# olegroshka/vae-channel-dynamics

Hardware: AMD Instinct MI355X
Metric: images/sec SDXL-VAE train step @256x256 (tracking on) (higher is better)
Workload: dtype f32

## Files before the change

vae-channel-dynamics_amd/csrc/conv3_upwino.hip:

```cpp
#include "wino_common.h"
#include <type_traits>
#include <algorithm>

#ifndef VAE_UPW_PRIO
#define VAE_UPW_PRIO 1
#endif

namespace {

constexpr int UTH = 4, UTW = 8;
constexpr int UTL = UTH * UTW;
static_assert(UTL == wino::TILES, "spill_acc");
constexpr int UBK = 8;
constexpr int NPOS = 9;
constexpr int UNT = 512;
constexpr int UNB = 2;
constexpr int USV = NPOS * UTL * UBK;
constexpr int UHF = (UTH + 2) * (UTW + 2);
constexpr int UHD = (2 * UTH + 2) * (2 * UTW + 2);
constexpr int USH = UHD * UBK;
constexpr int UMLD = 33;
constexpr int USM = NPOS * UTL * UMLD;
constexpr int UP_LDS = (USM > 2 * USV + 2 * USH ? USM : 2 * USV + 2 * USH) * 4;

__global__ __launch_bounds__(256) void upwino_weights_kernel(const float* __restrict__ W, int N, int K, int dgrad, int64_t sn, int64_t sk, int64_t st,
                                                             float* __restrict__ U) {
  const int64_t i = (int64_t)blockIdx.x * 256 + threadIdx.x;
  if (i >= (int64_t)N * K) return;
  const int k = (int)(i % K), n = (int)(i / K);
  float g[3][3];
  wino::u_gather(W, n, k, dgrad, sn, sk, st, g);
  float t[3][3];
#pragma unroll
  for (int b = 0; b < 3; ++b) {
    t[0][b] = g[0][b];
    t[1][b] = (g[0][b] + g[2][b]) + g[1][b];
    t[2][b] = g[2][b];
  }
  float* o = wino::u_out<NPOS>(U, N, n, k);
#pragma unroll
  for (int a = 0; a < 3; ++a) {
    wino::u_at(o, N, a * 3 + 0) = t[a][0];
    wino::u_at(o, N, a * 3 + 1) = (t[a][0] + t[a][2]) + t[a][1];
    wino::u_at(o, N, a * 3 + 2) = t[a][2];
  }
}

template <bool DG>
__global__ __launch_bounds__(UNT, 4) void conv3_upwino_kernel(vae_igemm_args p, const float* __restrict__ U, int tiles_x, int tiles_y, int xcd_sp) {
  constexpr int WBN = 32 * UNB;
  constexpr int HW_ = DG ? 2 * UTW + 2 : UTW + 2;
  constexpr int HP = DG ? UHD : UHF;
  __shared__ __attribute__((aligned(16))) float wsm[UP_LDS / 4];
  float* const sV = wsm;
  float* const sH = wsm + 2 * USV;

  const int tid = threadIdx.x, lane = tid & 63, wave = tid >> 6;
  const int xw0 = (blockIdx.x & 1) * 2;
  const bool extra = wave == xw0 || wave == xw0 + 1;
  const int xnb = wave - xw0;
  const int lr = lane & 31, lh = lane >> 5;
  const vae_conv_geom g = p.g;
  const int tilesN = (p.N + WBN - 1) / WBN;
  const wino::TileId wg = wino::tile_of_workgroup(blockIdx.x, tilesN, tiles_x, tiles_y, xcd_sp);
  const int b = wg.b;
  const int y0 = wg.ty * UTH, x0 = wg.tx * UTW, n0 = wg.tn * WBN;
  const int nsteps = p.K / UBK;

  const bool hrole = tid < 2 * HP;
  const int hp = tid >> 1, hq = tid & 1;
  const int hy = (DG ? 2 * y0 : y0) - 1 + hp / HW_, hx = (DG ? 2 * x0 : x0) - 1 + hp % HW_;
  const bool hin = hrole && ((unsigned)hy < (unsigned)g.Hs) && ((unsigned)hx < (unsigned)g.Ws);
  const auto rsA = VAE_BUF_RSRC(p.A + (int64_t)b * g.Hs * g.Ws * g.Cs, (size_t)g.Hs * g.Ws * g.Cs * 4u);
  const unsigned hbase = hin ? (unsigned)(((hy * g.Ws + hx) * g.Cs + hq * 4) * 4) : BUF_OOB;
  f32x4 rh = {0.f, 0.f, 0.f, 0.f};
  auto load_halo_into = [&](int step, f32x4& h) {
    const bool ok = hin && step < nsteps;
    h = VAE_BUF_LOAD4(rsA, ok ? hbase + (unsigned)(step * UBK * 4) : BUF_OOB);
  };
  auto store_halo_from = [&](float* dst, const f32x4& h) {
    if (hrole) *reinterpret_cast<f32x4*>(&dst[hp * UBK + hq * 4]) = h;
  };

  const bool vrole = tid < 256;
  const int vt = (tid >> 3) & 31, vc = tid & 7;
  const int vorg = DG ? ((2 * (vt >> 3)) * HW_ + 2 * (vt & 7)) * UBK + vc : ((vt >> 3) * HW_ + (vt & 7)) * UBK + vc;
  auto write_v = [&](const float* sHc, float* dst) {
    if (!vrole) return;
    float r[3][DG ? 4 : 3];
    if (!DG) {
      float d[3][3];
#pragma unroll
      for (int i = 0; i < 3; ++i)
#pragma unroll
        for (int j = 0; j < 3; ++j) d[i][j] = sHc[vorg + (i * HW_ + j) * UBK];
#pragma unroll
      for (int j = 0; j < 3; ++j) {
        r[0][j] = d[0][j] - d[1][j];
        r[1][j] = d[1][j];
        r[2][j] = d[1][j] - d[2][j];
      }
#pragma unroll
      for (int a = 0; a < 3; ++a) {
        dst[((a * 3 + 0) * UTL + vt) * UBK + vc] = r[a][0] - r[a][1];
        dst[((a * 3 + 1) * UTL + vt) * UBK + vc] = r[a][1];
        dst[((a * 3 + 2) * UTL + vt) * UBK + vc] = r[a][1] - r[a][2];
      }
    } else {
      float d[4][4];
#pragma unroll
      for (int i = 0; i < 4; ++i)
#pragma unroll
        for (int j = 0; j < 4; ++j) d[i][j] = sHc[vorg + (i * HW_ + j) * UBK];
#pragma unroll
      for (int j = 0; j < 4; ++j) {
        r[0][j] = d[0][j] - d[2][j];
        r[1][j] = d[1][j] + d[2][j];
        r[2][j] = d[1][j] - d[3][j];
      }
#pragma unroll
      for (int a = 0; a < 3; ++a) {
        dst[((a * 3 + 0) * UTL + vt) * UBK + vc] = r[a][0] - r[a][2];
        dst[((a * 3 + 1) * UTL + vt) * UBK + vc] = r[a][1] + r[a][2];
        dst[((a * 3 + 2) * UTL + vt) * UBK + vc] = r[a][1] - r[a][3];
      }
    }
  };

  const auto rsU = VAE_BUF_RSRC(U, wino::u_bytes(nsteps, NPOS, p.N));
  unsigned bvo[UNB];
#pragma unroll
  for (int q = 0; q < UNB; ++q) bvo[q] = (n0 + q * 32 + lr < p.N) ? wino::u_frag(n0 + q * 32 + lr, lh) : BUF_OOB;
  const unsigned bpos = wino::u_pos_bytes(p.N);
  const unsigned bvx = extra ? bvo[xnb & 1] : BUF_OOB;
  f32x4 bq[UNB + 1];
  auto load_b1 = [&](int step, int i) {
    const int st = min(step, nsteps - 1);
    const unsigned so = __builtin_amdgcn_readfirstlane((unsigned)(st * NPOS + (i < UNB ? wave : 8)) * bpos);
    bq[i] = __builtin_bit_cast(f32x4, __builtin_amdgcn_raw_buffer_load_b128(rsU, i < UNB ? bvo[i < UNB ? i : 0] : bvx, so, 0));
  };

  f32x16 acc[UNB], accx;
#pragma unroll
  for (int nb = 0; nb < UNB; ++nb)
#pragma unroll
    for (int e = 0; e < 16; ++e) acc[nb][e] = 0.f;
#pragma unroll
  for (int e = 0; e < 16; ++e) accx[e] = 0.f;

#pragma unroll
  for (int i = 0; i <= UNB; ++i) load_b1(0, i);
  {
    f32x4 h0, h1;
    load_halo_into(0, h0);
    load_halo_into(1, h1);
    load_halo_into(2, rh);
    store_halo_from(sH, h0);
    store_halo_from(sH + USH, h1);
  }
  __syncthreads();
  write_v(sH, sV);
  __syncthreads();
  auto multiply = [&](const float* cV, int s) {
    const f32x4 a4 = *reinterpret_cast<const f32x4*>(&cV[(wave * UTL + lr) * UBK + 4 * lh]);
    f32x4 ax = a4;
    if (extra) ax = *reinterpret_cast<const f32x4*>(&cV[(8 * UTL + lr) * UBK + 4 * lh]);
#pragma unroll
    for (int nb = 0; nb < UNB; ++nb) {
#pragma unroll
      for (int e = 0; e < 4; ++e) acc[nb] = __builtin_amdgcn_mfma_f32_32x32x2f32(a4[e], bq[nb][e], acc[nb], 0, 0, 0);
      __builtin_amdgcn_sched_barrier(0);
      load_b1(s + 1, nb);
      __builtin_amdgcn_sched_barrier(0);
    }
    if (extra) {
#pragma unroll
      for (int e = 0; e < 4; ++e) accx = __builtin_amdgcn_mfma_f32_32x32x2f32(ax[e], bq[UNB][e], accx, 0, 0, 0);
    }
    __builtin_amdgcn_sched_barrier(0);
    load_b1(s + 1, UNB);
    __builtin_amdgcn_sched_barrier(0);
  };
  auto stage_next = [&](int s, int par) {
    if (s + 1 < nsteps) write_v(sH + (par ^ 1) * USH, sV + (par ^ 1) * USV);
    store_halo_from(sH + par * USH, rh);
    load_halo_into(s + 3, rh);
  };
  auto step = [&](int s, int par, auto first_c) {
    const float* cV = sV + par * USV;
    if (decltype(first_c)::value) {
      stage_next(s, par);
      __builtin_amdgcn_sched_barrier(0);
      multiply(cV, s);
    } else {
      multiply(cV, s);
      __builtin_amdgcn_sched_barrier(0);
      stage_next(s, par);
    }
    __syncthreads();
  };
  auto run = [&](auto first_c) {
    int s = 0;
    for (; s + 1 < nsteps; s += 2) {
      step(s, 0, first_c);
      step(s + 1, 1, first_c);
    }
    if (s < nsteps) step(s, 0, first_c);
  };
#if VAE_UPW_PRIO
  if (DG && __builtin_amdgcn_readfirstlane(tid) >= 256) __builtin_amdgcn_s_setprio(1);
#endif
  if (wave < 4) run(std::true_type{});
  else run(std::false_type{});
#if VAE_UPW_PRIO
  if (DG) __builtin_amdgcn_s_setprio(0);
#endif

  float* const sM = wsm;
  const size_t obytes = (size_t)g.Ho * g.Wo * p.ldc * 4u;
  const auto rsC = VAE_BUF_RSRC(p.C + (int64_t)b * g.Ho * g.Wo * p.ldc, obytes);
#pragma unroll
  for (int nb = 0; nb < UNB; ++nb) {
    if (nb > 0) __syncthreads();
    wino::spill_acc(sM, wave, UMLD, acc[nb], lr, lh);
    if (wave == xw0 + nb) wino::spill_acc(sM, 8, UMLD, accx, lr, lh);
    __syncthreads();
    {
#pragma unroll
      for (int rnd = 0; rnd < 2; ++rnd) {
        const int co = tid & 31, tile = (tid >> 5) + 16 * rnd;
        const int col = n0 + nb * 32 + co;
        float m[9];
#pragma unroll
        for (int pos = 0; pos < 9; ++pos) m[pos] = sM[(pos * UTL + tile) * UMLD + co];
        const int oy = y0 + (tile >> 3), ox = x0 + (tile & 7);
        if (!DG) {
          const float bv = (p.bias && col < p.N) ? p.bias[col] : 0.f;
          float h[2][3];
#pragma unroll
          for (int j = 0; j < 3; ++j) {
            h[0][j] = m[0 * 3 + j] + m[1 * 3 + j];
            h[1][j] = m[1 * 3 + j] - m[2 * 3 + j];
          }
#pragma unroll
          for (int a = 0; a < 2; ++a) {
            const float yv[2] = {h[a][0] + h[a][1], h[a][1] - h[a][2]};
#pragma unroll
            for (int bb = 0; bb < 2; ++bb) {
              const int py = 2 * oy + a, px = 2 * ox + bb;
              const unsigned off = (col < p.N && py < g.Ho && px < g.Wo) ? (unsigned)(((py * g.Wo + px) * p.ldc + col) * 4) : BUF_OOB;
              __builtin_amdgcn_raw_buffer_store_b32(__builtin_bit_cast(unsigned, yv[bb] + bv), rsC, off, 0, 0);
            }
          }
        } else {
          const float h0 = (m[0] + m[3]) - m[6], h1 = (m[1] + m[4]) - m[7], h2 = (m[2] + m[5]) - m[8];
          const float v = (h0 + h1) - h2;
          const unsigned off = (col < p.N && oy < g.Ho && ox < g.Wo) ? (unsigned)(((oy * g.Wo + ox) * p.ldc + col) * 4) : BUF_OOB;
          __builtin_amdgcn_raw_buffer_store_b32(__builtin_bit_cast(unsigned, v), rsC, off, 0, 0);
        }
      }
    }
  }
}

}

bool conv3_upwino_eligible(const vae_igemm_args& a) {
  const vae_conv_geom& g = a.g;
  if (!wino::conv_eligible_common(a, NPOS) || a.xf != VAE_XF_NONE) return false;
  if (a.track != nullptr || a.res != nullptr || a.gstat != nullptr || a.a_bf16 || a.res_bf16) return false;
  int Hl, Wl;
  if (g.mode == VAE_MODE_UP2X) {
    if (g.Ho != 2 * g.Hs || g.Wo != 2 * g.Ws || a.sk != 1) return false;
    Hl = g.Hs; Wl = g.Ws;
  } else if (g.mode == VAE_MODE_UP2X_DGRAD) {
    if (g.Hs != 2 * g.Ho || g.Ws != 2 * g.Wo || a.sn != 1 || a.bias != nullptr) return false;
    Hl = g.Ho; Wl = g.Wo;
  } else {
    return false;
  }
  if (Hl % UTH != 0 || Wl % UTW != 0 || a.K % UBK != 0 || a.K < 64 || a.K > 1024 || a.N < 32 || a.N % 4 != 0 || g.Cs < a.K) return false;
  return true;
}

int launch_upwino_weights(const vae_igemm_args& a, float* U, hipStream_t st) {
  return wino::launch_weights(upwino_weights_kernel, a, a.g.mode == VAE_MODE_UP2X_DGRAD, U, st);
}

int launch_conv3_upwino(const vae_igemm_args& a, const float* U, hipStream_t st) {
  const vae_conv_geom& g = a.g;
  const bool dg = g.mode == VAE_MODE_UP2X_DGRAD;
  const int Hl = dg ? g.Ho : g.Hs, Wl = dg ? g.Wo : g.Ws;
  const int tx = Wl / UTW, ty = Hl / UTH;
  const int tilesN = (a.N + 32 * UNB - 1) / (32 * UNB);
  const int64_t nt = (int64_t)tilesN * tx * ty * g.B;
  if (nt > 0x7fffffffLL) return VAE_EINVAL;
  constexpr size_t xcd_u = (size_t)4 << 20;
  const int xcd_sp = wino::xcd_spatial(tilesN, wino::u_bytes(a.K / UBK, NPOS, a.N), xcd_u, (int64_t)tx * ty * g.B);
  if (dg) hipLaunchKernelGGL((conv3_upwino_kernel<true>), dim3((unsigned)nt), dim3(UNT), 0, st, a, U, tx, ty, xcd_sp);
  else hipLaunchKernelGGL((conv3_upwino_kernel<false>), dim3((unsigned)nt), dim3(UNT), 0, st, a, U, tx, ty, xcd_sp);
  return 0;
}
```

vae-channel-dynamics_amd/csrc/skinny.hip:

```cpp
#include "bf16_frag.h"
#include <algorithm>

namespace {

constexpr int TP = 128;
constexpr int NT = 256;
constexpr int TAPS_MAX = 9;

__device__ __forceinline__ void stage_small(const vae_conv_geom& g, const float* __restrict__ S, int Cs_small, int K, int m0,
                                            int mrows, f32x4* __restrict__ sI) {
  const int hw = g.Ho * g.Wo;
  const size_t sbytes = (size_t)g.B * g.Hs * g.Ws * Cs_small * 4u;
  const auto rsS = VAE_BUF_RSRC(S, sbytes < BUF_MAX ? sbytes : BUF_MAX);
  for (int e = threadIdx.x; e < TP * g.taps; e += NT) {
    const int row = e / g.taps, tap = e - row * g.taps;
    const int m = m0 + row;
    const int b = m / hw, rem = m - b * hw;
    const int y = rem / g.Wo, x = rem - y * g.Wo;
    const int kh = (g.taps == 9) ? tap / 3 : 0, kw = (g.taps == 9) ? tap - kh * 3 : 0;
    int sy = 0, sx = 0;
    const bool ok = (m < mrows) && src_pixel(g, y, x, kh, kw, sy, sx);
    const unsigned base = ok ? (unsigned)(((b * g.Hs + sy) * g.Ws + sx) * Cs_small) * 4u : BUF_OOB;
    f32x4 v = {0.f, 0.f, 0.f, 0.f};
#pragma unroll
    for (int s = 0; s < 4; ++s)
      if (s < K) v[s] = __builtin_bit_cast(float, __builtin_amdgcn_raw_buffer_load_b32(rsS, ok ? base + 4u * s : BUF_OOB, 0, 0));
    sI[e] = v;
  }
}

__global__ __launch_bounds__(NT) void conv_smallk_kernel(vae_igemm_args p) {
  __shared__ f32x4 sI[TP * TAPS_MAX];
  const vae_conv_geom g = p.g;
  const int tid = threadIdx.x, lane = tid & 127, half = tid >> 7;
  const int m0 = blockIdx.x * TP;
  const int n = blockIdx.y * 128 + lane;
  const bool nok = n < p.N;
  stage_small(g, p.A, g.Cs, p.K, m0, p.M, sI);

  float w[TAPS_MAX][4];
#pragma unroll
  for (int t = 0; t < TAPS_MAX; ++t)
#pragma unroll
    for (int s = 0; s < 4; ++s)
      w[t][s] = (nok && t < g.taps && s < p.K) ? p.W[(int64_t)n * p.sn + (int64_t)t * p.st + (int64_t)s * p.sk] : 0.f;
  const float bv = (p.bias && nok) ? p.bias[n] : 0.f;
  const bool cbf = p.out_bf16 != 0;
  const size_t obytes = (size_t)p.M * p.ldc * (cbf ? 2u : 4u);
  const auto rsC = VAE_BUF_RSRC(p.C, obytes);
  __syncthreads();

  float tsum = 0.f;
#pragma unroll 4
  for (int i = 0; i < TP / 2; ++i) {
    const int row = half + 2 * i;
    float acc = bv;
#pragma unroll
    for (int t = 0; t < TAPS_MAX; ++t) {
      if (t < g.taps) {
        const f32x4 v = sI[row * g.taps + t];
#pragma unroll
        for (int s = 0; s < 4; ++s) acc += v[s] * w[t][s];
      }
    }
    const int m = m0 + row;
    const bool ok = nok && m < p.M;
    buf_store1_elem(rsC, cbf, ok ? m * p.ldc + n : -1, acc);
    const float stored = cbf ? (float)(__bf16)acc : acc;
    tsum += ok ? fabsf(stored) : 0.f;
  }
  if (p.track) {
    __syncthreads();
    float* red = reinterpret_cast<float*>(sI);
    red[tid] = tsum;
    __syncthreads();
    if (half == 0 && nok) p.track[(int64_t)blockIdx.x * p.N + n] = red[lane] + red[128 + lane];
  }
}

template <bool SMALL_X, int XF>
__global__ __launch_bounds__(NT) void wgrad_smallk_kernel(vae_wgrad_args p, vae_conv_geom gs, int ntiles) {
  __shared__ f32x4 sI[TP * TAPS_MAX + 32];
  const int tid = threadIdx.x, lane = tid & 127, half = tid >> 7;
  const int split = blockIdx.x;
  const int ch = blockIdx.y * 128 + lane;
  const int wide = SMALL_X ? p.M : p.N, narrow = SMALL_X ? p.N : p.M;
  const bool chok = ch < wide;
  const float* __restrict__ V = SMALL_X ? p.dY : p.X;
  const float* __restrict__ S = SMALL_X ? p.X : p.dY;
  const int ldv = SMALL_X ? p.ldy : p.g.Cs, lds_ = SMALL_X ? p.g.Cs : p.ldy;
  const int npixv = gs.B * gs.Ho * gs.Wo;
  const int hwv = gs.Ho * gs.Wo;
  const bool vbf = (SMALL_X ? p.y_bf16 : p.x_bf16) != 0;
  const size_t vbytes = (size_t)npixv * ldv * (vbf ? 2u : 4u);
  const auto rsV = VAE_BUF_RSRC(V, vbytes < BUF_MAX ? vbytes : BUF_MAX);

  float acc[TAPS_MAX][4];
#pragma unroll
  for (int t = 0; t < TAPS_MAX; ++t)
#pragma unroll
    for (int s = 0; s < 4; ++s) acc[t][s] = 0.f;
  float vsum = 0.f;
  f32x4 ssum = {0.f, 0.f, 0.f, 0.f};
  int xb = -1;
  float xsc = 1.f, xsh = 0.f;

  const int per = (ntiles + p.nsplit - 1) / p.nsplit;
  const int tbeg = split * per, tend = min(ntiles, tbeg + per);
  for (int tile = tbeg; tile < tend; ++tile) {
    const int m0 = tile * TP;
    __syncthreads();
    stage_small(gs, S, lds_, narrow, m0, npixv, sI);
    __syncthreads();
#pragma unroll 4
    for (int i = 0; i < TP / 2; ++i) {
      const int row = half + 2 * i;
      const int m = m0 + row;
      const bool ok = chok && m < npixv;
      float v = buf_load1_elem(rsV, vbf, ok ? m * ldv + ch : -1);
      if (XF != VAE_XF_NONE) {
        const int b = min(m, npixv - 1) / hwv;
        if (b != xb) {
          xb = b;
          xsc = chok ? p.scale[(int64_t)b * p.g.Cs + ch] : 0.f;
          xsh = chok ? p.shift[(int64_t)b * p.g.Cs + ch] : 0.f;
        }
        float u = v * xsc + xsh;
        if (XF == VAE_XF_AFFINE_SILU) u = silu_f(u);
        v = ok ? u : 0.f;
      }
      if (SMALL_X) vsum += v;
#pragma unroll
      for (int t = 0; t < TAPS_MAX; ++t) {
        if (t < gs.taps) {
          const f32x4 sv = sI[row * gs.taps + t];
#pragma unroll
          for (int s = 0; s < 4; ++s) acc[t][s] += v * sv[s];
          if (!SMALL_X && t == gs.taps / 2) ssum += sv;
        }
      }
    }
  }

  __syncthreads();
  float* red = reinterpret_cast<float*>(sI);
  if (half == 1) {
#pragma unroll
    for (int t = 0; t < TAPS_MAX; ++t)
#pragma unroll
      for (int s = 0; s < 4; ++s) red[lane * 36 + t * 4 + s] = acc[t][s];
    if (SMALL_X) red[128 * 36 + lane] = vsum;
    else if (lane == 0) {
#pragma unroll
      for (int s = 0; s < 4; ++s) red[128 * 36 + s] = ssum[s];
    }
  }
  __syncthreads();
  if (half == 0) {
    const int64_t ld = (int64_t)gs.taps * p.N;
    float* __restrict__ O = (p.nsplit == 1 ? p.out : p.partial + (int64_t)split * p.M * ld);
    if (chok) {
#pragma unroll
      for (int t = 0; t < TAPS_MAX; ++t)
#pragma unroll
        for (int s = 0; s < 4; ++s)
          if (t < gs.taps && s < narrow) {
            const float r = acc[t][s] + red[lane * 36 + t * 4 + s];
            if (SMALL_X) O[(int64_t)ch * ld + (int64_t)t * p.N + s] = p.alpha * r;
            else O[(int64_t)s * ld + (int64_t)t * p.N + ch] = p.alpha * r;
          }
    }
    if (p.bias_partial) {
      if (SMALL_X) {
        if (chok) p.bias_partial[(int64_t)split * p.M + ch] = vsum + red[128 * 36 + lane];
      } else if (blockIdx.y == 0 && lane < p.M) {
        p.bias_partial[(int64_t)split * p.M + lane] = ssum[lane] + red[128 * 36 + lane];
      }
    }
  }
}

}

bool conv_smallk_eligible(const vae_igemm_args& a) {
  const vae_conv_geom& g = a.g;
  return a.K <= 4 && a.batch == 1 && a.xf == VAE_XF_NONE && a.res == nullptr && a.alpha == 1.0f && g.taps <= TAPS_MAX &&
         g.mode != VAE_MODE_DGRAD_S2 && (size_t)a.M * a.ldc * 4u < BUF_MAX && (size_t)g.B * g.Hs * g.Ws * g.Cs * 4u < BUF_MAX;
}
int launch_conv_smallk(const vae_igemm_args& a, hipStream_t st) {
  dim3 grid((unsigned)((a.M + TP - 1) / TP), (unsigned)((a.N + 127) / 128));
  hipLaunchKernelGGL(conv_smallk_kernel, grid, dim3(NT), 0, st, a);
  return 0;
}

int wgrad_smallk_kind(const vae_wgrad_args& a) {
  const vae_conv_geom& g = a.g;
  if (a.batch != 1 || g.taps > TAPS_MAX) return 0;
  if ((size_t)a.npix * a.ldy * 4u >= BUF_MAX || (size_t)g.B * g.Hs * g.Ws * g.Cs * 4u >= BUF_MAX) return 0;
  if (a.N <= 4 && a.xf == VAE_XF_NONE && (g.mode == VAE_MODE_FWD || g.mode == VAE_MODE_UP2X)) return 1;
  if (a.M <= 4 && g.mode == VAE_MODE_FWD && g.stride == 1 && g.Ho == g.Hs && g.Wo == g.Ws &&
      ((g.taps == 9 && g.pad_t == 1 && g.pad_l == 1) || (g.taps == 1 && g.pad_t == 0 && g.pad_l == 0)))
    return 2;
  return 0;
}
int wgrad_smallk_tiles(const vae_wgrad_args& a) { return (int)(((int64_t)a.g.B * a.g.Ho * a.g.Wo + TP - 1) / TP); }
static vae_conv_geom wgrad_smallk_geom(const vae_wgrad_args& a, int kind) {
  vae_conv_geom gs = a.g;
  if (kind == 2) {
    gs.mode = VAE_MODE_DGRAD;
    gs.Cs = a.ldy;
  }
  return gs;
}
int launch_wgrad_thin_bf16(const vae_wgrad_args& a, int kind, const vae_conv_geom& gs, int ntiles, hipStream_t st);
int launch_wgrad_thin(const vae_wgrad_args& a, hipStream_t st) {
  const int kind = wgrad_smallk_kind(a);
  return launch_wgrad_thin_bf16(a, kind, wgrad_smallk_geom(a, kind), wgrad_smallk_tiles(a), st);
}

int launch_wgrad_smallk(const vae_wgrad_args& a, hipStream_t st) {
  const int kind = wgrad_smallk_kind(a);
  const int ntiles = wgrad_smallk_tiles(a);
  const vae_conv_geom gs = wgrad_smallk_geom(a, kind);
  const int wide = kind == 1 ? a.M : a.N;
  dim3 grid((unsigned)a.nsplit, (unsigned)((wide + 127) / 128));
#define WSK(SX, XFV) hipLaunchKernelGGL((wgrad_smallk_kernel<SX, XFV>), grid, dim3(NT), 0, st, a, gs, ntiles)
  if (kind == 1) WSK(true, VAE_XF_NONE);
  else if (a.xf == VAE_XF_NONE) WSK(false, VAE_XF_NONE);
  else if (a.xf == VAE_XF_AFFINE) WSK(false, VAE_XF_AFFINE);
  else WSK(false, VAE_XF_AFFINE_SILU);
#undef WSK
  return 0;
}

namespace {

constexpr int NTH = 4, NTW = 32, NHW = NTW + 2, NHP = (NTH + 2) * NHW;
constexpr int NBK = 32, NLD = NBK + 4, NNT = 128;
constexpr int NHQ = NHP * (NBK / 4), NHI = (NHQ + NNT - 1) / NNT;

template <int XF>
__global__ __launch_bounds__(NNT) void conv_smalln_kernel(vae_igemm_args p, int tiles_x, int tiles_y) {
  __shared__ __attribute__((aligned(16))) float sH[NHP * NLD];
  const vae_conv_geom g = p.g;
  const int tid = threadIdx.x;
  int t = blockIdx.x;
  const int tx = t % tiles_x; t /= tiles_x;
  const int ty = t % tiles_y;
  const int b = t / tiles_y;
  const int y0 = ty * NTH, x0 = tx * NTW;
  const int pr = tid >> 5, px = tid & 31;
  const bool abf = p.a_bf16 != 0;
  const unsigned esA = abf ? 2u : 4u;
  const auto rsA = VAE_BUF_RSRC(reinterpret_cast<const char*>(p.A) + (int64_t)b * g.Hs * g.Ws * g.Cs * esA, (size_t)g.Hs * g.Ws * g.Cs * esA);
  const float* __restrict__ W = p.W;

  float acc[4] = {0.f, 0.f, 0.f, 0.f};
  const int hk4 = tid & 7;
  uint4 rh[NHI];
  int hmask = 0;
  f32x4 rsc = {0.f, 0.f, 0.f, 0.f}, rsh = {0.f, 0.f, 0.f, 0.f};
  auto load_halo = [&](int c0) {
    hmask = 0;
    const int c = c0 + hk4 * 4;
    if (XF != VAE_XF_NONE) {
      const int cs = min(c, p.K - 4);
      rsc = *reinterpret_cast<const f32x4*>(p.scale + (int64_t)b * g.Cs + cs);
      rsh = *reinterpret_cast<const f32x4*>(p.shift + (int64_t)b * g.Cs + cs);
    }
#pragma unroll
    for (int i = 0; i < NHI; ++i) {
      const int q = tid + NNT * i;
      const int pp = q >> 3;
      const int ir = pp / NHW, jc = pp - ir * NHW;
      const int hy = y0 - 1 + ir, hx = x0 - 1 + jc;
      const bool ok = (q < NHQ) && ((unsigned)hy < (unsigned)g.Hs) && ((unsigned)hx < (unsigned)g.Ws) && (c < p.K);
      rh[i] = buf_load4_raw(rsA, esA, ok ? ((hy * g.Ws + hx) * g.Cs + c) : -1);
      hmask |= (ok ? 1 : 0) << i;
    }
  };
  auto store_halo = [&]() {
#pragma unroll
    for (int i = 0; i < NHI; ++i) {
      const int q = tid + NNT * i;
      if (q < NHQ) {
        f32x4 v = raw4_to_f32(rh[i], abf);
        if (XF != VAE_XF_NONE) {
          const bool ok = (hmask >> i) & 1;
#pragma unroll
          for (int e = 0; e < 4; ++e) {
            float u = v[e] * rsc[e] + rsh[e];
            if (XF == VAE_XF_AFFINE_SILU) u = silu_f(u);
            v[e] = ok ? u : 0.f;
          }
        }
        *reinterpret_cast<f32x4*>(&sH[(q >> 3) * NLD + hk4 * 4]) = v;
      }
    }
  };

  const int kchunks = (p.K + NBK - 1) / NBK;
  load_halo(0);
  for (int cch = 0; cch < kchunks; ++cch) {
    const int c0 = cch * NBK;
    __syncthreads();
    store_halo();
    __syncthreads();
    if (cch + 1 < kchunks) load_halo(c0 + NBK);
#pragma unroll
    for (int tap = 0; tap < 9; ++tap) {
      const int kh = tap / 3, kw = tap - kh * 3;
      const float* hrow = &sH[((pr + kh) * NHW + px + kw) * NLD];
#pragma unroll
      for (int q = 0; q < NBK / 4; ++q) {
        const f32x4 a = *reinterpret_cast<const f32x4*>(hrow + q * 4);
#pragma unroll
        for (int s = 0; s < 4; ++s) {
          if (s < p.N) {
            const f32x4 w4 = *reinterpret_cast<const f32x4*>(W + (int64_t)s * p.sn + (int64_t)tap * p.st + c0 + q * 4);
#pragma unroll
            for (int e = 0; e < 4; ++e) acc[s] = __builtin_fmaf(a[e], w4[e], acc[s]);
          }
        }
      }
    }
  }

  const int oy = y0 + pr, ox = x0 + px;
  const auto rsC = VAE_BUF_RSRC(p.C + (int64_t)b * g.Ho * g.Wo * p.ldc, (size_t)g.Ho * g.Wo * p.ldc * 4u);
#pragma unroll
  for (int s = 0; s < 4; ++s)
    if (s < p.N) {
      const float v = acc[s] + (p.bias ? p.bias[s] : 0.f);
      __builtin_amdgcn_raw_buffer_store_b32(__builtin_bit_cast(unsigned, v), rsC,
                                            (oy < g.Ho && ox < g.Wo) ? (unsigned)(((oy * g.Wo + ox) * p.ldc + s) * 4) : BUF_OOB, 0, 0);
    }
}

}

bool conv_smalln_eligible(const vae_igemm_args& a) {
  const vae_conv_geom& g = a.g;
  return a.N <= 4 && a.K >= NBK && a.K % NBK == 0 && a.sn % 4 == 0 && a.st % 4 == 0 && aligned16(a.W) && a.batch == 1 && a.res == nullptr && a.track == nullptr && a.alpha == 1.0f &&
         a.A16 == nullptr && g.mode == VAE_MODE_FWD && g.taps == 9 && g.stride == 1 && g.pad_t == 1 && g.pad_l == 1 &&
         g.Ho == g.Hs && g.Wo == g.Ws && g.Wo % NTW == 0 && g.Ho % NTH == 0 && a.sk == 1 && g.Cs % 4 == 0 && aligned16(a.A) &&
         (a.xf == VAE_XF_NONE || (aligned16(a.scale) && aligned16(a.shift))) &&
         (size_t)g.Hs * g.Ws * g.Cs * 4u < BUF_MAX && (size_t)g.Ho * g.Wo * a.ldc * 4u < BUF_MAX;
}
int launch_conv_smalln(const vae_igemm_args& a, hipStream_t st) {
  const int tx = a.g.Wo / NTW, ty = a.g.Ho / NTH;
  dim3 grid((unsigned)((int64_t)tx * ty * a.g.B));
  switch (a.xf) {
    case VAE_XF_NONE: hipLaunchKernelGGL((conv_smalln_kernel<VAE_XF_NONE>), grid, dim3(NNT), 0, st, a, tx, ty); break;
    case VAE_XF_AFFINE: hipLaunchKernelGGL((conv_smalln_kernel<VAE_XF_AFFINE>), grid, dim3(NNT), 0, st, a, tx, ty); break;
    default: hipLaunchKernelGGL((conv_smalln_kernel<VAE_XF_AFFINE_SILU>), grid, dim3(NNT), 0, st, a, tx, ty); break;
  }
  return 0;
}
```

Before: 108.8.

## Assign extra winograd wave by SIMD seat and pipeline small-K conv/wgrad staging

The upsample winograd kernel now picks which waves handle the extra ninth position from each wave's hardware SIMD id, read via s_getreg and shared through LDS, so the extra MFMA work lands on distinct SIMDs. It also adds optional timing instrumentation behind a macro. The small-K conv kernel gets templated tap-specialized staging, and the wgrad small-K kernel gets a double-buffered software pipeline that prefetches the next tile and batches row loads. These changes add LDS, register pressure and code complexity, and the SIMD-id mapping relies on hardware register layout.

```diff
diff --git a/vae-channel-dynamics_amd/csrc/conv3_upwino.hip b/vae-channel-dynamics_amd/csrc/conv3_upwino.hip
--- a/vae-channel-dynamics_amd/csrc/conv3_upwino.hip
+++ b/vae-channel-dynamics_amd/csrc/conv3_upwino.hip
@@ -4,6 +4,10 @@
 
 #ifndef VAE_UPW_PRIO
 #define VAE_UPW_PRIO 1
+#endif
+
+#ifndef VAE_UPW_SEAT
+#define VAE_UPW_SEAT 2
 #endif
 
 namespace {
@@ -56,9 +60,19 @@
   float* const sH = wsm + 2 * USV;
 
   const int tid = threadIdx.x, lane = tid & 63, wave = tid >> 6;
-  const int xw0 = (blockIdx.x & 1) * 2;
-  const bool extra = wave == xw0 || wave == xw0 + 1;
-  const int xnb = wave - xw0;
+#if VAE_UPW_SEAT == 0
+  const int slot = blockIdx.x & 1;
+#else
+  const int slot = __builtin_amdgcn_s_getreg(6 | (11 << 11)) != 0;
+#endif
+  int seat = (2 * slot) | ((2 * slot + 1) << 2);
+#if VAE_UPW_SEAT == 2
+  int* const sSeat = reinterpret_cast<int*>(wsm + 2 * USV + 2 * USH);
+  static_assert(2 * USV + 2 * USH + 4 <= UP_LDS / 4, "sSeat");
+  if (tid < 256 && lane == 0) sSeat[wave] = __builtin_amdgcn_s_getreg(4 | (4 << 6) | (1 << 11));
+#endif
+  int xws0 = 0, xws1 = 0, xnb = 0;
+  bool extra = false;
   const int lr = lane & 31, lh = lane >> 5;
   const vae_conv_geom g = p.g;
   const int tilesN = (p.N + WBN - 1) / WBN;
@@ -132,7 +146,17 @@
 #pragma unroll
   for (int q = 0; q < UNB; ++q) bvo[q] = (n0 + q * 32 + lr < p.N) ? wino::u_frag(n0 + q * 32 + lr, lh) : BUF_OOB;
   const unsigned bpos = wino::u_pos_bytes(p.N);
-  const unsigned bvx = extra ? bvo[xnb & 1] : BUF_OOB;
+  unsigned bvx = BUF_OOB;
+  auto take_seat = [&]() {
+    xws0 = seat & 3;
+    xws1 = seat >> 2;
+    extra = wave == xws0 || wave == xws1;
+    xnb = wave == xws1;
+    bvx = extra ? bvo[xnb & 1] : BUF_OOB;
+  };
+#if VAE_UPW_SEAT != 2
+  take_seat();
+#endif
   f32x4 bq[UNB + 1];
   auto load_b1 = [&](int step, int i) {
     const int st = min(step, nsteps - 1);
@@ -149,7 +173,7 @@
   for (int e = 0; e < 16; ++e) accx[e] = 0.f;
 
 #pragma unroll
-  for (int i = 0; i <= UNB; ++i) load_b1(0, i);
+  for (int i = 0; i < (VAE_UPW_SEAT == 2 ? UNB : UNB + 1); ++i) load_b1(0, i);
   {
     f32x4 h0, h1;
     load_halo_into(0, h0);
@@ -159,6 +183,20 @@
     store_halo_from(sH + USH, h1);
   }
   __syncthreads();
+#if VAE_UPW_SEAT == 2
+  {
+    int at = 0, seen = 0;
+#pragma unroll
+    for (int w = 0; w < 4; ++w) {
+      const int sd = __builtin_amdgcn_readfirstlane(sSeat[w]) & 3;
+      at |= w << (2 * sd);
+      seen |= 1 << sd;
+    }
+    if (seen == 15) seat = (at >> (4 * slot)) & 15;
+    take_seat();
+    load_b1(0, UNB);
+  }
+#endif
   write_v(sH, sV);
   __syncthreads();
   auto multiply = [&](const float* cV, int s) {
@@ -186,18 +224,31 @@
     store_halo_from(sH + par * USH, rh);
     load_halo_into(s + 3, rh);
   };
+#ifdef VAE_UPW_TIMING
+  unsigned tMul = 0u, tBar = 0u, tFirst = 0u, tLast = 0u, tN = 0u, tA = 0u;
+#define UPW_STAMP(s, k) do { if ((s) >= 2) { const unsigned t_ = (unsigned)__builtin_amdgcn_s_memtime(); \
+    if ((k) == 0) { if (tN == 0u) tFirst = t_; } else if ((k) == 1) tMul += t_ - tA; else if ((k) == 3) { tBar += t_ - tA; tLast = t_; ++tN; } tA = t_; } } while (0)
+#else
+#define UPW_STAMP(s, k) do { } while (0)
+#endif
   auto step = [&](int s, int par, auto first_c) {
     const float* cV = sV + par * USV;
     if (decltype(first_c)::value) {
       stage_next(s, par);
       __builtin_amdgcn_sched_barrier(0);
+      UPW_STAMP(s, 0);
       multiply(cV, s);
+      UPW_STAMP(s, 1);
     } else {
+      UPW_STAMP(s, 0);
       multiply(cV, s);
+      UPW_STAMP(s, 1);
       __builtin_amdgcn_sched_barrier(0);
       stage_next(s, par);
     }
+    UPW_STAMP(s, 2);
     __syncthreads();
+    UPW_STAMP(s, 3);
   };
   auto run = [&](auto first_c) {
     int s = 0;
@@ -216,6 +267,13 @@
   if (DG) __builtin_amdgcn_s_setprio(0);
 #endif
 
+#ifdef VAE_UPW_TIMING
+  if (p.track && blockIdx.x < 256 && lane == 0) {
+    unsigned* o = reinterpret_cast<unsigned*>(p.track) + (blockIdx.x * 8 + wave) * 8;
+    o[0] = tMul; o[1] = tBar; o[2] = tLast - tFirst; o[3] = tN;
+    o[4] = __builtin_amdgcn_s_getreg(4 | (4 << 6) | (1 << 11)); o[5] = extra ? 1u : 0u; o[6] = (unsigned)slot; o[7] = (unsigned)(xws0 | (xws1 << 2));
+  }
+#endif
   float* const sM = wsm;
   const size_t obytes = (size_t)g.Ho * g.Wo * p.ldc * 4u;
   const auto rsC = VAE_BUF_RSRC(p.C + (int64_t)b * g.Ho * g.Wo * p.ldc, obytes);
@@ -223,7 +281,7 @@
   for (int nb = 0; nb < UNB; ++nb) {
     if (nb > 0) __syncthreads();
     wino::spill_acc(sM, wave, UMLD, acc[nb], lr, lh);
-    if (wave == xw0 + nb) wino::spill_acc(sM, 8, UMLD, accx, lr, lh);
+    if (wave == (nb ? xws1 : xws0)) wino::spill_acc(sM, 8, UMLD, accx, lr, lh);
     __syncthreads();
     {
 #pragma unroll
@@ -268,7 +326,10 @@
 bool conv3_upwino_eligible(const vae_igemm_args& a) {
   const vae_conv_geom& g = a.g;
   if (!wino::conv_eligible_common(a, NPOS) || a.xf != VAE_XF_NONE) return false;
-  if (a.track != nullptr || a.res != nullptr || a.gstat != nullptr || a.a_bf16 || a.res_bf16) return false;
+#ifndef VAE_UPW_TIMING
+  if (a.track != nullptr) return false;
+#endif
+  if (a.res != nullptr || a.gstat != nullptr || a.a_bf16 || a.res_bf16) return false;
   int Hl, Wl;
   if (g.mode == VAE_MODE_UP2X) {
     if (g.Ho != 2 * g.Hs || g.Wo != 2 * g.Ws || a.sk != 1) return false;
diff --git a/vae-channel-dynamics_amd/csrc/skinny.hip b/vae-channel-dynamics_amd/csrc/skinny.hip
--- a/vae-channel-dynamics_amd/csrc/skinny.hip
+++ b/vae-channel-dynamics_amd/csrc/skinny.hip
@@ -29,6 +29,38 @@
   }
 }
 
+template <int TAPS>
+__device__ __forceinline__ void stage_small_load(const SrcMap& sm, __amdgpu_buffer_rsrc_t rsS, int Cs_small, int K, int hw, int Wo, int m0, int mrows,
+                                                 f32x4 (&v)[(TAPS + 1) / 2]) {
+  static_assert(TAPS == 9 || TAPS == 1, "kh, kw below");
+  const int row = threadIdx.x >> 1, h = threadIdx.x & 1;
+  const int m = m0 + row;
+  const int b = m / hw, rem = m - b * hw;
+  const int y = rem / Wo, x = rem - y * Wo;
+#pragma unroll
+  for (int k = 0; k < (TAPS + 1) / 2; ++k) {
+    const int tap = h + 2 * k;
+    const int kh = TAPS == 9 ? (tap * 11) >> 5 : 0, kw = TAPS == 9 ? tap - 3 * kh : 0;
+    int sy = 0, sx = 0;
+    const bool ok = (tap < TAPS) && (m < mrows) && src_pixel(sm, y, x, kh, kw, sy, sx);
+    const unsigned base = oob_unless(ok, (unsigned)(((b * sm.Hs + sy) * sm.Ws + sx) * Cs_small) * 4u);
+#pragma unroll
+    for (int s = 0; s < 4; ++s)
+      v[k][s] = __builtin_bit_cast(float, __builtin_amdgcn_raw_buffer_load_b32(rsS, s < K ? base + 4u * s : BUF_OOB, 0, 0));
+  }
+}
+template <int TAPS>
+__device__ __forceinline__ void stage_small_store(f32x4* __restrict__ sI, const f32x4 (&v)[(TAPS + 1) / 2]) {
+  const int row = threadIdx.x >> 1, h = threadIdx.x & 1;
+#pragma unroll
+  for (int k = 0; k < (TAPS + 1) / 2; ++k)
+    if (h + 2 * k < TAPS) sI[row * TAPS + h + 2 * k] = v[k];
+}
+__device__ __forceinline__ auto small_rsrc(const vae_conv_geom& g, const float* S, int Cs_small) {
+  const size_t sbytes = (size_t)g.B * g.Hs * g.Ws * Cs_small * 4u;
+  return VAE_BUF_RSRC(S, sbytes < BUF_MAX ? sbytes : BUF_MAX);
+}
+
 __global__ __launch_bounds__(NT) void conv_smallk_kernel(vae_igemm_args p) {
   __shared__ f32x4 sI[TP * TAPS_MAX];
   const vae_conv_geom g = p.g;
@@ -36,7 +68,21 @@
   const int m0 = blockIdx.x * TP;
   const int n = blockIdx.y * 128 + lane;
   const bool nok = n < p.N;
-  stage_small(g, p.A, g.Cs, p.K, m0, p.M, sI);
+  if (g.taps == 9 || g.taps == 1) {
+    const SrcMap sm = make_srcmap(g);
+    const auto rsS = small_rsrc(g, p.A, g.Cs);
+    if (g.taps == 9) {
+      f32x4 st[5];
+      stage_small_load<9>(sm, rsS, g.Cs, p.K, g.Ho * g.Wo, g.Wo, m0, p.M, st);
+      stage_small_store<9>(sI, st);
+    } else {
+      f32x4 st[1];
+      stage_small_load<1>(sm, rsS, g.Cs, p.K, g.Ho * g.Wo, g.Wo, m0, p.M, st);
+      stage_small_store<1>(sI, st);
+    }
+  } else {
+    stage_small(g, p.A, g.Cs, p.K, m0, p.M, sI);
+  }
 
   float w[TAPS_MAX][4];
 #pragma unroll
@@ -78,10 +124,101 @@
   }
 }
 
+template <bool SMALL_X, int XF, int NS, int TAPS>
+__device__ __forceinline__ void wgrad_smallk_tiles(const vae_wgrad_args& p, const vae_conv_geom& gs, f32x4* __restrict__ sI, int tbeg, int tend, int ch,
+                                                   bool chok, int half, float (&acc)[TAPS_MAX][4], float& vsum, f32x4& ssum) {
+  constexpr int G = 8, NG = TP / 2 / G, SB = TP * TAPS;
+  const float* __restrict__ V = SMALL_X ? p.dY : p.X;
+  const float* __restrict__ S = SMALL_X ? p.X : p.dY;
+  const int narrow = SMALL_X ? p.N : p.M;
+  const int ldv = SMALL_X ? p.ldy : p.g.Cs, lds_ = SMALL_X ? p.g.Cs : p.ldy;
+  const int npixv = gs.B * gs.Ho * gs.Wo, hwv = gs.Ho * gs.Wo;
+  const size_t vbytes = (size_t)npixv * ldv * 4u;
+  const auto rsV = VAE_BUF_RSRC(V, vbytes < BUF_MAX ? vbytes : BUF_MAX);
+  const auto rsS = small_rsrc(gs, S, lds_);
+  const SrcMap sm = make_srcmap(gs);
+  if (tbeg >= tend) return;
+
+  f32x4 st[(TAPS + 1) / 2];
+  float vc[G], vn[G];
+  auto load_rows = [&](int mfirst, float (&v)[G]) {
+#pragma unroll
+    for (int j = 0; j < G; ++j) {
+      const int m = mfirst + 2 * j;
+      v[j] = __builtin_bit_cast(float, __builtin_amdgcn_raw_buffer_load_b32(rsV, oob_unless(chok && m < npixv, (unsigned)(m * ldv + ch) * 4u), 0, 0));
+    }
+  };
+  stage_small_load<TAPS>(sm, rsS, lds_, narrow, hwv, gs.Wo, tbeg * TP, npixv, st);
+  load_rows(tbeg * TP + half, vc);
+  stage_small_store<TAPS>(sI, st);
+  __syncthreads();
+
+  int xrun = (tbeg * TP + half) / hwv, xrem = (tbeg * TP + half) - xrun * hwv;
+  int xb = -1;
+  float xsc = 1.f, xsh = 0.f;
+  for (int tile = tbeg; tile < tend; ++tile) {
+    const int m0 = tile * TP, par = (tile - tbeg) & 1;
+    const f32x4* __restrict__ cI = sI + par * SB;
+    const bool more = tile + 1 < tend;
+    if (more) stage_small_load<TAPS>(sm, rsS, lds_, narrow, hwv, gs.Wo, m0 + TP, npixv, st);
+#pragma unroll 1
+    for (int gq = 0; gq < NG; ++gq) {
+      float sc[G], sh[G];
+      if (XF != VAE_XF_NONE) {
+        const bool plain = xrem + 2 * (G - 1) < hwv && min(xrun, gs.B - 1) == xb;
+        if (plain) {
+#pragma unroll
+          for (int j = 0; j < G; ++j) { sc[j] = xsc; sh[j] = xsh; }
+        } else {
+          int lb = xrun, lrem = xrem;
+#pragma unroll
+          for (int j = 0; j < G; ++j) {
+            const int b = min(lb, gs.B - 1);
+            if (b != xb) {
+              xb = b;
+              xsc = chok ? p.scale[(int64_t)b * p.g.Cs + ch] : 0.f;
+              xsh = chok ? p.shift[(int64_t)b * p.g.Cs + ch] : 0.f;
+            }
+            sc[j] = xsc; sh[j] = xsh;
+            lrem += 2;
+            while (lrem >= hwv) { lrem -= hwv; ++lb; }
+          }
+          __builtin_amdgcn_s_waitcnt(0x0F70);
+        }
+        xrem += 2 * G;
+        while (xrem >= hwv) { xrem -= hwv; ++xrun; }
+      }
+      load_rows(m0 + half + 2 * G * (gq + 1), vn);
+#pragma unroll
+      for (int j = 0; j < G; ++j) {
+        const int row = half + 2 * (gq * G + j);
+        float v = vc[j];
+        if (XF != VAE_XF_NONE) {
+          float u = v * sc[j] + sh[j];
+          if (XF == VAE_XF_AFFINE_SILU) u = silu_f(u);
+          v = (chok && m0 + row < npixv) ? u : 0.f;
+        }
+        if (SMALL_X) vsum += v;
+#pragma unroll
+        for (int t = 0; t < TAPS; ++t) {
+          const f32x4 sv = cI[row * TAPS + t];
+#pragma unroll
+          for (int s = 0; s < NS; ++s) acc[t][s] += v * sv[s];
+          if (!SMALL_X && t == TAPS / 2) ssum += sv;
+        }
+      }
+#pragma unroll
+      for (int j = 0; j < G; ++j) vc[j] = vn[j];
+    }
+    if (more) stage_small_store<TAPS>(sI + (par ^ 1) * SB, st);
+    __syncthreads();
+  }
+}
+
 template <bool SMALL_X, int XF>
 __global__ __launch_bounds__(NT) void wgrad_smallk_kernel(vae_wgrad_args p, vae_conv_geom gs, int ntiles) {
-  __shared__ f32x4 sI[TP * TAPS_MAX + 32];
-  const int tid = threadIdx.x, lane = tid & 127, half = tid >> 7;
+  __shared__ f32x4 sI[2 * TP * TAPS_MAX + 32];
+  const int tid = threadIdx.x, lane = tid & 127, half = __builtin_amdgcn_readfirstlane(tid >> 7);
   const int split = blockIdx.x;
   const int ch = blockIdx.y * 128 + lane;
   const int wide = SMALL_X ? p.M : p.N, narrow = SMALL_X ? p.N : p.M;
@@ -107,7 +244,17 @@
 
   const int per = (ntiles + p.nsplit - 1) / p.nsplit;
   const int tbeg = split * per, tend = min(ntiles, tbeg + per);
-  for (int tile = tbeg; tile < tend; ++tile) {
+  const bool piped = !vbf && (gs.taps == 9 || gs.taps == 1);
+  if (piped) {
+    if (gs.taps == 9) {
+      if (narrow == 3) wgrad_smallk_tiles<SMALL_X, XF, 3, 9>(p, gs, sI, tbeg, tend, ch, chok, half, acc, vsum, ssum);
+      else wgrad_smallk_tiles<SMALL_X, XF, 4, 9>(p, gs, sI, tbeg, tend, ch, chok, half, acc, vsum, ssum);
+    } else {
+      if (narrow == 3) wgrad_smallk_tiles<SMALL_X, XF, 3, 1>(p, gs, sI, tbeg, tend, ch, chok, half, acc, vsum, ssum);
+      else wgrad_smallk_tiles<SMALL_X, XF, 4, 1>(p, gs, sI, tbeg, tend, ch, chok, half, acc, vsum, ssum);
+    }
+  }
+  for (int tile = piped ? tend : tbeg; tile < tend; ++tile) {
     const int m0 = tile * TP;
     __syncthreads();
     stage_small(gs, S, lds_, narrow, m0, npixv, sI);
```

Result: no change. 109.8 (median of 6 runs) (+0.9%).
